# maelaubert/VulkanSift

Hardware: AMD Instinct MI355X
Metric: SIFT detect+match frames/sec (640x480, ~2k kp) (higher is better)
Workload: dtype f32

## Files before the change

include/vksift_hip.h:

```cpp
#ifndef VKSIFT_HIP_H
#define VKSIFT_HIP_H

#include <stddef.h>
#include <stdint.h>

#ifdef __cplusplus
extern "C"
{
#endif

#define VKSIFT_HIP_MAX_TAPS 20
#define VKSIFT_HIP_MATCH_CHUNKS 32
#define VKSIFT_HIP_MATCH_SMALL_NA 1536u
#define VKSIFT_HIP_MATCH_SMALL_NB 4096u
#define VKSIFT_HIP_MATCH_SCRATCH_U32(na, nb) (2u * (size_t)(na) + (size_t)(nb) + 72u + (size_t)(na) * 16u * VKSIFT_HIP_MATCH_CHUNKS)
#define VKSIFT_HIP_ABI_VERSION 14u
#define VKSIFT_HIP_GATHER_SLOTS 512u
#define VKSIFT_HIP_MATCH_SLOTS 256u
#define VKSIFT_HIP_MATCH_PK_NB 32768u
#define VKSIFT_HIP_MAX_ORI 18
#define VKSIFT_HIP_MAX_OCTAVE_SIDE 16383u

  typedef void *vksift_hip_stream;
  typedef void *vksift_hip_graph;
  typedef void *vksift_hip_event;

  int vksift_hip_init(void);
  uint32_t vksift_hip_abi_version(void);
  int vksift_hip_device_count(void);
  int vksift_hip_device_name(int idx, char *out256);
  int vksift_hip_set_device(int idx);
  size_t vksift_hip_device_free_mem(void);
  void *vksift_hip_malloc(size_t bytes);
  void vksift_hip_free(void *p);
  void *vksift_hip_host_malloc(size_t bytes);
  void vksift_hip_host_free(void *p);
  int vksift_hip_host_register(void *p, size_t bytes);
  int vksift_hip_host_unregister(void *p);
  int vksift_hip_is_pinned(const void *p);
  vksift_hip_stream vksift_hip_stream_create(void);
  void vksift_hip_stream_destroy(vksift_hip_stream s);
  int vksift_hip_stream_sync(vksift_hip_stream s);
  int vksift_hip_stream_busy(vksift_hip_stream s);
  vksift_hip_event vksift_hip_event_create(void);
  void vksift_hip_event_destroy(vksift_hip_event e);
  int vksift_hip_event_record(vksift_hip_event e, vksift_hip_stream s);
  int vksift_hip_event_sync(vksift_hip_event e);
  int vksift_hip_event_busy(vksift_hip_event e);
  float vksift_hip_event_elapsed_ms(vksift_hip_event a, vksift_hip_event b);
  int vksift_hip_stream_wait_event(vksift_hip_stream s, vksift_hip_event e);
  int vksift_hip_capture_begin(vksift_hip_stream s);
  int vksift_hip_capture_end(vksift_hip_stream s, vksift_hip_graph *out);
  int vksift_hip_graph_launch(vksift_hip_graph g, vksift_hip_stream s);
  void vksift_hip_graph_destroy(vksift_hip_graph g);
  int vksift_hip_memcpy_h2d(void *dst, const void *src, size_t n, vksift_hip_stream s);
  int vksift_hip_memcpy_d2h(void *dst, const void *src, size_t n, vksift_hip_stream s);
  int vksift_hip_memcpy_d2d(void *dst, const void *src, size_t n, vksift_hip_stream s);
  int vksift_hip_memcpy2d_d2h(void *dst, size_t dpitch, const void *src, size_t spitch, size_t width_bytes, size_t height, vksift_hip_stream s);
  int vksift_hip_post_words(uint32_t *host_mapped_dst, const uint32_t *src, size_t n_words, vksift_hip_stream s);
  int vksift_hip_memset(void *dst, int value, size_t n, vksift_hip_stream s);
  const char *vksift_hip_error_string(int err);
  void vksift_hip_range_push(const char *name);
  void vksift_hip_range_pop(void);

  enum
  {
    VKSIFT_TUNE_WG_TARGET = 0,
    VKSIFT_TUNE_WIDE_MASK = 1,
    VKSIFT_TUNE_MULTI_MAX = 2,
    VKSIFT_TUNE_REFINE_PTR = 3,
    VKSIFT_TUNE_SCAN_FORM = 4,
    VKSIFT_TUNE_PAIR_FORM = 5,
    VKSIFT_TUNE_PYR_GATE = 6,
    VKSIFT_TUNE_DENSE_ROWS = 7,
    VKSIFT_TUNE_SEED_WG = 8,
    VKSIFT_TUNE_SCAN_BAND = 9,
    VKSIFT_TUNE_TAIL_MULTI = 10,
    VKSIFT_TUNE_ZERO_COPY = 11,
    VKSIFT_TUNE_MIN_MARCH = 12,
    VKSIFT_TUNE_TAIL_FUSED = 13,
    VKSIFT_TUNE_COUNT = 16
  };
  int vksift_hip_tune(int knob, int value);
  int vksift_hip_tune_get(int knob);


  typedef struct
  {
    float *base;
    uint32_t w, h;
    uint32_t pitch;
    uint64_t img_stride;
    uint32_t fp16;
    uint32_t reverse;
  } vksift_hip_Plane;

  int vksift_hip_input_blit(const uint8_t *src, uint32_t sw, uint32_t sh, uint64_t src_img_stride, vksift_hip_Plane dst, uint32_t batch,
                            vksift_hip_stream s);

  int vksift_hip_blur(vksift_hip_Plane src, vksift_hip_Plane dst, const float *taps, uint32_t ntaps, uint32_t batch, vksift_hip_stream s);

  int vksift_hip_blur_pair(vksift_hip_Plane src, vksift_hip_Plane dst1, vksift_hip_Plane dst2, const float *taps1, uint32_t ntaps1, const float *taps2,
                           uint32_t ntaps2, uint32_t batch, vksift_hip_stream s);

  int vksift_hip_blur_form(vksift_hip_Plane src, vksift_hip_Plane dst, uint32_t ntaps, uint32_t batch);

  int vksift_hip_blur_multi(const vksift_hip_Plane *src, const vksift_hip_Plane *dst, uint32_t n, const float *taps, uint32_t ntaps, uint32_t batch,
                            vksift_hip_stream s);

  int vksift_hip_blur_downsample(vksift_hip_Plane src, vksift_hip_Plane dst, vksift_hip_Plane next, const float *taps, uint32_t ntaps, uint32_t batch,
                                 vksift_hip_stream s);

  int vksift_hip_seed_upsampled(const uint8_t *src, uint32_t sw, uint32_t sh, uint64_t src_img_stride, vksift_hip_Plane dst, const float *taps, uint32_t ntaps,
                                uint32_t batch, vksift_hip_stream s);

  int vksift_hip_seed_direct(const uint8_t *src, uint32_t sw, uint32_t sh, uint64_t src_img_stride, vksift_hip_Plane dst, const float *taps, uint32_t ntaps,
                             uint32_t batch, vksift_hip_stream s);

  int vksift_hip_downsample(vksift_hip_Plane src, vksift_hip_Plane dst, uint32_t batch, vksift_hip_stream s);

  int vksift_hip_octave_chain(const vksift_hip_Plane *layers, uint32_t n_oct, uint32_t n_layers, uint32_t S, const float *taps, const uint32_t *ntaps,
                              uint32_t batch, vksift_hip_stream s);

  int vksift_hip_dog_plane(const float *lo, const float *hi, uint32_t w, uint32_t h, uint32_t pitch, uint32_t fp16, float *out_dense, vksift_hip_stream s);

  typedef struct
  {
    float *gauss;
    uint32_t fp16;
    uint32_t w, h, pitch;
    uint64_t plane_stride;
    uint64_t img_stride;
    uint32_t S;
    int32_t octave_idx;
    float seed_sigma;
    float dog_threshold;
    float edge_limit;
    uint8_t *feats;
    uint64_t feat_img_stride;
    uint32_t cap;
    uint32_t *found;
    uint32_t found_img_stride;
    uint64_t *seg_mask;
    uint32_t *seg_off;
    uint64_t seg_img_stride;
    uint32_t *cand_xy;
    uint32_t *cand_flag;
    uint32_t *cand_n;
    uint64_t cand_img_stride;
    uint32_t cand_cap;
    float *ori_ang;
    uint32_t *ori_cnt;
    uint64_t ori_img_stride;
    uint32_t max_ori;
    uint32_t use_vlfeat;
    const float *desc_fp_tab;
    uint32_t desc_fp_tab_len;
    uint32_t scan_reverse;
    uint32_t masks_cleared;
    uint32_t sec_index;
  } vksift_hip_OctaveJob;

  typedef struct
  {
    uint8_t *desc;
    uint64_t desc_img_stride;
    uint32_t *norm;
    uint64_t norm_img_stride;
    uint32_t *n;
    uint32_t n_img_stride;
    uint32_t nsec;
    uint32_t sec_cap[16];
    uint8_t *post;
    uint64_t post_img_stride;
    uint32_t *found_post;
    uint32_t found_post_n;
  } vksift_hip_DenseRows;

  int vksift_hip_extract_keypoints(const vksift_hip_OctaveJob *job, uint32_t batch, vksift_hip_stream s, vksift_hip_event scan_done);
  int vksift_hip_orientations(const vksift_hip_OctaveJob *job, uint32_t batch, vksift_hip_stream s);
  int vksift_hip_descriptors(const vksift_hip_OctaveJob *job, uint32_t batch, vksift_hip_stream s);
  int vksift_hip_extract_keypoints_multi(const vksift_hip_OctaveJob *jobs, uint32_t n_jobs, uint32_t batch, vksift_hip_stream s, vksift_hip_event scan_done);
  int vksift_hip_clear_segment_masks(const vksift_hip_OctaveJob *jobs, uint32_t n_jobs, uint32_t batch, vksift_hip_stream s);
  int vksift_hip_selftest_inrange(uint32_t n, uint32_t seed, uint32_t *d_mismatches, vksift_hip_stream s);
  int vksift_hip_orientations_multi(const vksift_hip_OctaveJob *jobs, uint32_t n_jobs, uint32_t batch, vksift_hip_stream s);
  int vksift_hip_descriptors_multi(const vksift_hip_OctaveJob *jobs, uint32_t n_jobs, uint32_t batch, vksift_hip_stream s);
  int vksift_hip_descriptors_multi_dense(const vksift_hip_OctaveJob *jobs, uint32_t n_jobs, uint32_t batch, const vksift_hip_DenseRows *dense,
                                         vksift_hip_stream s);

  typedef struct
  {
    float x, y, sigma, orientation, response;
  } vksift_hip_Keypoint;
  typedef struct
  {
    uint32_t w, h;
    int32_t octave_idx;
    uint8_t *feats;
    uint64_t feat_img_stride;
    uint32_t cap;
    uint32_t *found;
    uint32_t found_img_stride;
  } vksift_hip_PlaceOctave;
#define VKSIFT_HIP_PLACE_WG 256u
  int vksift_hip_place_keypoints(const vksift_hip_Keypoint *kps, const uint32_t *kp_first, const vksift_hip_PlaceOctave *oct, uint32_t n_oct,
                                 const float *sigma_steps, uint32_t S, uint32_t keep_orientation, uint32_t batch, uint32_t *placed, vksift_hip_stream s);

  int vksift_hip_gather_descriptors(const uint8_t *feats, uint32_t n, uint8_t *desc, vksift_hip_stream s);
  size_t vksift_hip_match_scratch_u32(uint32_t na, uint32_t nb);
  int vksift_hip_match_2nn_desc(const uint8_t *desc_a, uint32_t na, uint32_t a_index_base, const uint8_t *desc_b, uint32_t nb, uint32_t *norm_scratch,
                                size_t scratch_u32, uint8_t *matches, vksift_hip_stream s);
  int vksift_hip_shifted_norms(const uint8_t *desc, uint32_t n, uint32_t *norms, vksift_hip_stream s);
  int vksift_hip_match_2nn_prenormed(const uint8_t *desc_a, const uint32_t *norm_a, uint32_t na, uint32_t a_index_base, const uint8_t *desc_b,
                                     const uint32_t *norm_b, uint32_t nb, uint32_t *scratch, size_t scratch_u32, uint8_t *matches, vksift_hip_stream s);

  int vksift_hip_filter_matches(const uint8_t *fwd, uint64_t fwd_slot_stride, const uint8_t *rev, uint64_t rev_slot_stride, const uint32_t *n_fwd,
                                uint32_t n_stride, float ratio, uint32_t nslots, uint8_t *out, uint64_t out_slot_stride, uint32_t *out_n, vksift_hip_stream s);

  int vksift_hip_pack_features(const uint8_t *feats_base, uint64_t buf_stride, const uint32_t *buf_ids, const uint32_t *out_rows, uint32_t nslots, uint32_t nsec,
                               const uint32_t *sec_off, const uint32_t *sec_cap, const uint32_t *found_base, uint32_t found_buf_stride, uint8_t *out,
                               uint32_t max_rows, uint32_t *found_post, vksift_hip_stream s);
  int vksift_hip_gather_sections(const uint8_t *feats_base, uint64_t buf_stride, const uint32_t *buf_ids, uint32_t nslots, uint32_t nsec,
                                 const uint32_t *sec_off, const uint32_t *sec_cap, const uint32_t *fixed_counts, const uint32_t *found_base,
                                 uint32_t found_buf_stride, uint32_t max_rows, uint32_t pad_rows_to, uint8_t *desc, uint64_t desc_stride,
                                 uint32_t *norms, uint64_t norm_stride, uint32_t *n_out_dev, uint32_t n_stride, vksift_hip_stream s);
  int vksift_hip_keep_strongest(uint8_t *feats_base, uint64_t buf_stride, const uint32_t *buf_ids, uint32_t nslots, uint32_t nsec, const uint32_t *sec_off,
                                const uint32_t *sec_cap, const uint32_t *fixed_counts, uint32_t *found_base, uint32_t found_buf_stride, uint32_t *found_post,
                                uint32_t max_features, uint32_t pad_rows_to, uint8_t *desc, uint64_t desc_stride, uint32_t *norms, uint64_t norm_stride,
                                uint32_t *n_out_dev, uint32_t n_stride, vksift_hip_stream s);
  int vksift_hip_keep_grid(uint8_t *feats_base, uint64_t buf_stride, const uint32_t *buf_ids, uint32_t nslots, uint32_t nsec, const uint32_t *sec_off,
                           const uint32_t *sec_cap, const uint32_t *fixed_counts, uint32_t *found_base, uint32_t found_buf_stride, uint32_t *found_post,
                           uint32_t max_features, uint32_t grid_cols, uint32_t grid_rows, const float *col_bounds, const float *row_bounds,
                           uint32_t pad_rows_to, uint8_t *desc, uint64_t desc_stride, uint32_t *norms, uint64_t norm_stride, uint32_t *n_out_dev,
                           uint32_t n_stride, vksift_hip_stream s);
  int vksift_hip_root_descriptors(uint8_t *feats_base, uint64_t buf_stride, const uint32_t *buf_ids, uint32_t nslots, uint32_t nsec, const uint32_t *sec_off,
// ... 59 lines not shown
```

vulkansift_amd/csrc/hip/features.hip:

```cpp
#include <hip/hip_runtime.h>
#include <stdint.h>
#include <stdlib.h>
#include <type_traits>

#include "../detmath.h"
#include "features_math.h"
#include "multi.h"
#include "records.h"
#include "vksift_hip.h"
#include "wave.h"

namespace
{

struct FeatArgs
{
  const float *gauss;
  uint32_t fp16;
  int w, h, pitch;
  uint64_t plane_stride, img_stride;
  uint8_t *feats;
  uint64_t feat_img_stride;
  uint32_t cap;
  uint32_t *found;
// ... 167 lines not shown
      }
      uint32_t hm = __shfl(hv, lm, 64), hp = __shfl(hv, lp, 64);
      const uint32_t mx = wave_max_u32(lane < 36 ? hv : 0u);
      bool peak = lane < 36 && ((float)hv >= (0.8f * (float)mx)) && (hv > hm) && (hv > hp);
      unsigned long long pm = __ballot(peak);
      uint32_t npk = (uint32_t)__popcll(pm);
      if (peak)
      {
        uint32_t rank = ballot_rank(pm, lane);
        if (rank < a.max_keep)
        {
          uint32_t num = hm - hp;
          uint32_t den = hm - (2u * hv) + hp;
          float idx = (float)lane + 0.5f * ((float)num / (float)den);
          float ang = (idx + 0.5f) * (2.f * PI_F) / 36.f;
          a.ori_ang[((size_t)b * a.ori_img_stride + k) * VKSIFT_HIP_MAX_ORI + rank] = ang;
        }
      }
      if (lane == 0)
        a.ori_cnt[(size_t)b * a.ori_img_stride + k] = npk < a.max_keep ? npk : a.max_keep;
    }
    __builtin_amdgcn_wave_barrier();
  }
}

__global__ void __launch_bounds__(1024) k_orientation_finalize(Multi<FeatArgs> m)
{
  __shared__ uint32_t wave_tot[16];
  __shared__ uint32_t carry_s;
  const VBlock vb = vblock(m);
  const FeatArgs &a = m.oct[vb.o];
  const int b = (int)vb.x;
  const int lane = threadIdx.x & 63, wave = threadIdx.x >> 6;
  const ImageView g = image_view(a, b);
  const uint32_t *cnt = a.ori_cnt + (size_t)b * a.ori_img_stride;
  const float *ang = a.ori_ang + (size_t)b * a.ori_img_stride * VKSIFT_HIP_MAX_ORI;
  if (threadIdx.x == 0)
    carry_s = 0;
  __syncthreads();
  for (uint32_t base = 0; base < g.n; base += 1024)
  {
    uint32_t k = base + threadIdx.x;
    uint32_t c = k < g.n ? cnt[k] : 0u;
    uint32_t v = c > 1 ? c - 1 : 0u;
    const uint32_t incl = wave_scan_incl_u32(v, lane);
    if (lane == 63)
      wave_tot[wave] = incl;
    __syncthreads();
    uint32_t wave_base = 0;
    for (int wv = 0; wv < wave; wv++)
      wave_base += wave_tot[wv];
    uint32_t carry = carry_s;
    uint32_t excl = carry + wave_base + incl - v;
    if (k < g.n && c >= 1)
    {
      uint32_t *rec = (uint32_t *)(g.feats + (size_t)k * VKSIFT_RECORD_BYTES);
      rec[7] = __float_as_uint(ang[(size_t)k * VKSIFT_HIP_MAX_ORI]);
      for (uint32_t j = 1; j < c; j++)
      {
        uint32_t idx = g.found + excl + (j - 1);
        if (idx < a.cap)
        {
          uint32_t *dst = (uint32_t *)(g.feats + (size_t)idx * VKSIFT_RECORD_BYTES);
#pragma unroll
          for (int q = 0; q < (int)VKSIFT_RECORD_HEAD_WORDS; q++)
            dst[q] = rec[q];
          dst[7] = __float_as_uint(ang[(size_t)k * VKSIFT_HIP_MAX_ORI + j]);
        }
      }
    }
    __syncthreads();
    if (threadIdx.x == 1023)
      carry_s = carry + wave_base + incl;
    __syncthreads();
  }
  if (threadIdx.x == 0)
    a.found[(size_t)b * a.found_img_stride] = g.found + carry_s;
}

__device__ __forceinline__ int smod8(int v) { return v & 7; }

struct DescCtx
{
  __amdgpu_buffer_rsrc_t rs;
  int pitch, pitch4;
  float scale_x, scale_y, rsx, rsy, kcos, ksin, kori, fp, bin_scale;
  int dx0, dx1, dy0, dy1;
  float offx, offy, ia0, ia1;
};

struct DescSample
{
  float ox, oy, mag;
  float xb;
};

struct DescTaps
{
  float up, lf, rt, dn;
};

__device__ __forceinline__ unsigned desc_tap_base(const DescCtx &c, int cdx, int cdy)
{
  const int ix = (int)c.rsx + cdx, iy = (int)c.rsy + cdy;
  return (__umul24((unsigned)(iy - 1), (unsigned)c.pitch) + (unsigned)(ix - 1)) * 4u;
}

template <bool F16>
__device__ __forceinline__ DescTaps desc_taps(const DescCtx &c, unsigned v0)
{
  DescTaps t;
  t.up = tap_ld<F16>(c.rs, v0 + 4u, 0);
  t.lf = tap_ld<F16>(c.rs, v0, c.pitch4);
  t.rt = tap_ld<F16>(c.rs, v0 + 8u, c.pitch4);
  t.dn = tap_ld<F16>(c.rs, v0 + 4u, 2 * c.pitch4);
  return t;
}

typedef uint32_t u32x2_t __attribute__((ext_vector_type(2)));
typedef uint32_t u32x4_t __attribute__((ext_vector_type(4)));
__device__ __forceinline__ void desc_taps_pair(const DescCtx &c, unsigned v0, DescTaps &a, DescTaps &b)
{
  const u32x2_t up = __builtin_amdgcn_raw_buffer_load_b64(c.rs, v0 + 4u, 0, 0);
  const u32x4_t mid = __builtin_amdgcn_raw_buffer_load_b128(c.rs, v0, c.pitch4, 0);
  const u32x2_t dn = __builtin_amdgcn_raw_buffer_load_b64(c.rs, v0 + 4u, 2 * c.pitch4, 0);
  a.up = __uint_as_float(up.x), b.up = __uint_as_float(up.y);
  a.lf = __uint_as_float(mid.x), b.lf = __uint_as_float(mid.y);
  a.rt = __uint_as_float(mid.z), b.rt = __uint_as_float(mid.w);
  a.dn = __uint_as_float(dn.x), b.dn = __uint_as_float(dn.y);
}

template <bool INRANGE>
__device__ __forceinline__ DescSample desc_sample(const DescCtx &c, int cdx, int cdy, const DescTaps &t, bool *odd)
{
  const float es = -1.f / (2.f * 2 * 2);
  float sdx = (c.rsx + (float)cdx) - c.scale_x;
  float sdy = (c.rsy + (float)cdy) - c.scale_y;
  DescSample r;
  r.ox = c.kcos * sdx + c.ksin * sdy;
  r.oy = c.kcos * sdy - c.ksin * sdx;
  float gradX = 0.5f * (t.rt - t.lf);
  float gradY = 0.5f * (t.dn - t.up);
  float ori, root;
  grad_polar<INRANGE>(gradX, gradY, &ori, &root, odd);
  ori = wrap_2pi(ori);
  ori = wrap_2pi(ori - c.kori);
  r.mag = dm_expf_core_nonpos(es * ((r.ox * r.ox) + (r.oy * r.oy))) * root;
  r.xb = ori * c.bin_scale;
  return r;
}

constexpr int DESC_PAD = 1, DESC_ROW_CELLS = 8;
constexpr int DESC_HIST_WORDS = (4 + 2 * DESC_PAD) * DESC_ROW_CELLS * 16;
constexpr int DESC_WORK_WORDS = DESC_HIST_WORDS;
__device__ __forceinline__ int desc_cell_word(int cell)
{
  return (((cell >> 2) + DESC_PAD) * DESC_ROW_CELLS + (cell & 3) + DESC_PAD) * 16;
}
__device__ __forceinline__ uint32_t desc_hist_read(const uint32_t *s_work, int t)
{
  const int cw = desc_cell_word(t >> 3), bin = t & 7;
  return s_work[cw + 2 * bin] + s_work[cw + 2 * ((bin + 7) & 7) + 1];
}

__device__ __forceinline__ void desc_scatter(const DescCtx &c, const DescSample &r, float fbin, bool live, uint32_t *s_work)
{
  float fhx = r.ox + 2.f, fhy = r.oy + 2.f;
  const float flx = floorf(fhx - 0.5f), fly = floorf(fhy - 0.5f), flb = floorf(fbin);
  int hx = (int)flx, hy = (int)fly, hb = (int)flb;
  float rhx = fhx - (flx + 0.5f), rhy = fhy - (fly + 0.5f), rb = fbin - flb;
  const float magfp = r.mag * c.fp;
  const unsigned b0 = (unsigned)smod8(hb);
  const unsigned pair = b0 * 8u;
  const bool okx[2] = {live && (unsigned)hx < 4u, live && (unsigned)(hx + 1) < 4u};
  const bool oky[2] = {(unsigned)hy < 4u, (unsigned)(hy + 1) < 4u};
  char *base = (char *)s_work + ((unsigned)((hy + DESC_PAD) * (DESC_ROW_CELLS * 64) + (hx + DESC_PAD) * 64) + pair);
#pragma unroll
  for (int i = 0; i < 2; i++)
#pragma unroll
    for (int j = 0; j < 2; j++)
    {
      const float w = fabsf(1.f - (float)i - rhx) * fabsf(1.f - (float)j - rhy);
      const uint32_t v0 = (uint32_t)((w * fabsf(1.f - 0.f - rb)) * magfp);
      const uint32_t v1 = (uint32_t)((w * fabsf(1.f - 1.f - rb)) * magfp);
      if (okx[i] && oky[j])
        atomicAdd((unsigned long long *)(base + (j * DESC_ROW_CELLS * 64 + i * 64)), ((unsigned long long)v1 << 32) | v0);
    }
}

constexpr int DESC_MAX_ROWS = 256;

template <bool CAN_POST>
__device__ __forceinline__ void desc_dense_prologue(const FeatArgs &a, const vksift_hip_DenseRows &dr, int b, bool first_block, int tid, uint32_t *s_row0)
{
  if (!(dr.desc || (CAN_POST && dr.post)))
    return;
  const uint32_t *fsec = a.found + (size_t)b * a.found_img_stride - a.sec;
  uint32_t row0 = 0, total = 0;
#pragma unroll
  for (uint32_t j = 0; j < 16u; j++)
    if (j < dr.nsec)
    {
      const uint32_t f = fsec[j], n = f < dr.sec_cap[j] ? f : dr.sec_cap[j];
      row0 += j < a.sec ? n : 0u;
      total += n;
    }
  if (tid == 0)
    *s_row0 = row0;
  if (a.sec == 0 && first_block)
  {
    if (CAN_POST && dr.post && (uint32_t)tid < dr.found_post_n)
      dr.found_post[(size_t)b * dr.found_post_n + tid] = fsec[tid];
    if (dr.desc && tid == 0)
      dr.n[(size_t)b * dr.n_img_stride] = total;
    if (dr.desc && total < 2u && tid < 64)
    {
      uint32_t *z = (uint32_t *)(dr.desc + (size_t)b * dr.desc_img_stride);
      if (tid >= (int)total * 32)
        z[tid] = 0u;
      if (tid < 2 && tid >= (int)total)
        dr.norm[(size_t)b * dr.norm_img_stride + tid] = 128u * 128u * 128u;
    }
  }
}

__device__ __forceinline__ DescCtx desc_setup(const FeatArgs &a, const ImageView &g, const KeyHead &kh)
{
  DescCtx c;
  c.scale_x = kh.scale_x, c.scale_y = kh.scale_y, c.kori = kh.theta;
  c.rs = kh.rs;
  c.pitch = g.pitch, c.pitch4 = g.pitch * 4;
  c.bin_scale = a.use_vlfeat ? 8.f : -8.f;
  float scale_factor = dm_pow2i(kh.octave_idx);
  float lambda = 3.0f * (kh.sigma / scale_factor);
  float radius = sqrtf(2.f) * lambda * 5.f * 0.5f;
  int R = (int)floorf(radius + 0.5f);
  float sn, cs;
  dm_sincosf(c.kori, &sn, &cs);
  c.kcos = cs / lambda, c.ksin = sn / lambda;
  uint32_t ti = (uint32_t)(R / 2);
  c.fp = a.desc_fp_tab[ti < a.desc_fp_tab_len ? ti : a.desc_fp_tab_len - 1];
  c.rsx = roundf(c.scale_x), c.rsy = roundf(c.scale_y);

  const int cxi = (int)c.rsx, cyi = (int)c.rsy;
  c.dx0 = max(-R, 1 - cxi), c.dx1 = min(R, g.w - 2 - cxi);
  c.dy0 = max(-R, 1 - cyi), c.dy1 = min(R, g.h - 2 - cyi);
  c.offx = c.rsx - c.scale_x, c.offy = c.rsy - c.scale_y;
  c.ia0 = __builtin_amdgcn_rcpf(c.kcos), c.ia1 = __builtin_amdgcn_rcpf(-c.ksin);
  return c;
}

struct DescRows
{
  int *lo;
  uint32_t *cnt;
  const uint32_t *pre;
  int y0, nrows;
};

template <int NT>
__device__ __forceinline__ void desc_row_spans(const DescCtx &c, const DescRows &rows, int tid)
{
  const float T = 2.5f + 0.01f;
  for (int row = tid; row < rows.nrows; row += NT)
  {
    const float fy = (float)(rows.y0 + row) + c.offy;
    float lo = (float)c.dx0 - 0.5f, hi = (float)c.dx1 + 0.5f;
#pragma unroll
    for (int e = 0; e < 2; e++)
    {
      const float aa = e == 0 ? c.kcos : -c.ksin, ia = e == 0 ? c.ia0 : c.ia1;
      const float bb = e == 0 ? c.ksin * fy : c.kcos * fy;
      if (fabsf(aa) > 1e-12f)
      {
        const float ctr = -bb * ia - c.offx, half = T * fabsf(ia);
        lo = fmaxf(lo, ctr - half);
        hi = fminf(hi, ctr + half);
      }
      else if (!(fabsf(bb) < T))
        hi = lo - 2.f;
    }
    const int ilo = (int)ceilf(lo - 0.01f), ihi = (int)floorf(hi + 0.01f);
    const int xl = max(ilo, c.dx0), xh = min(ihi, c.dx1);
    rows.lo[row] = xl;
    rows.cnt[row] = xh >= xl ? (uint32_t)(xh - xl + 1) : 0u;
  }
}

__device__ __forceinline__ void desc_row_prefix(const DescRows &rows, uint32_t *pre, int lane)
{
  uint32_t carry = 0;
  for (int base = 0; base < rows.nrows; base += 64)
  {
    const int i = base + lane;
    const uint32_t v = i < rows.nrows ? rows.cnt[i] : 0u;
    const uint32_t incl = wave_scan_incl_u32(v, lane);
    if (i < rows.nrows)
      pre[i] = carry + incl - v;
    carry += __shfl(incl, 63, 64);
  }
  if (lane == 0)
    pre[rows.nrows] = carry;
}

struct DescRun
{
  uint32_t steps;
  uint32_t sidx, send;
  int row, cdx;
  uint32_t row_end;
};
template <int NWV>
__device__ __forceinline__ DescRun desc_run(const DescRows &rows, int wave, int lane)
{
  const uint32_t *s_pre = rows.pre;
  const uint32_t N = s_pre[rows.nrows];
  const uint32_t T = (N + 63u) / 64u, tq = T / NWV, tr = T % NWV;
  DescRun r;
  r.steps = tq + ((uint32_t)wave < tr ? 1u : 0u);
  const uint32_t step0 = (uint32_t)wave * tq + min((uint32_t)wave, tr);
  r.sidx = min(N, step0 * 64u + (uint32_t)lane * r.steps);
  r.send = min(N, r.sidx + r.steps);
  int row = 0;
  if (r.sidx < r.send)
  {
    int lo_r = 0, hi_r = rows.nrows - 1;
    while (lo_r < hi_r)
    {
      const int mid = (lo_r + hi_r + 1) >> 1;
      if (s_pre[mid] <= r.sidx)
        lo_r = mid;
      else
        hi_r = mid - 1;
    }
    row = lo_r;
    while (s_pre[row + 1] <= r.sidx)
      row++;
  }
  r.row = row;
  r.cdx = rows.lo[row] + (int)(r.sidx - s_pre[row]);
  r.row_end = s_pre[row + 1];
  return r;
}

__device__ __forceinline__ bool desc_next_sample(const DescRows &rows, DescRun &r, int &sx, int &sy)
{
  const bool live = r.sidx < r.send;
  if (live && r.sidx >= r.row_end)
  {
    do
      r.row++;
    while (rows.pre[r.row + 1] <= r.sidx);
    r.row_end = rows.pre[r.row + 1];
    r.cdx = rows.lo[r.row];
  }
  sx = r.cdx, sy = rows.y0 + r.row;
  r.cdx++, r.sidx++;
  return live;
}

template <bool F16>
__device__ __forceinline__ void desc_step_pair(const DescCtx &c, const DescRows &rows, DescRun &run, uint32_t *s_work)
{
  int sx[2], sy[2];
  const bool live[2] = {desc_next_sample(rows, run, sx[0], sy[0]), desc_next_sample(rows, run, sx[1], sy[1])};
  DescTaps t0, t1;
  const unsigned v0 = desc_tap_base(c, sx[0], sy[0]);
  if (F16)
  {
    t0 = desc_taps<F16>(c, v0);
    t1 = desc_taps<F16>(c, desc_tap_base(c, sx[1], sy[1]));
  }
  else
  {
    desc_taps_pair(c, v0, t0, t1);
    if (live[1] && !(sy[1] == sy[0] && sx[1] == sx[0] + 1))
      t1 = desc_taps<F16>(c, desc_tap_base(c, sx[1], sy[1]));
  }
  bool o0, o1;
  DescSample s0 = desc_sample<true>(c, sx[0], sy[0], t0, &o0), s1 = desc_sample<true>(c, sx[1], sy[1], t1, &o1);
  float f0 = angle_bin<true>(s0.xb), f1 = angle_bin<true>(s1.xb);
  o0 |= angle_bin_odd(s0.xb), o1 |= angle_bin_odd(s1.xb);
  if (__builtin_expect(__ballot(o0 || o1) != 0ull, 0))
  {
    s0 = desc_sample<false>(c, sx[0], sy[0], t0, nullptr), s1 = desc_sample<false>(c, sx[1], sy[1], t1, nullptr);
    f0 = angle_bin<false>(s0.xb), f1 = angle_bin<false>(s1.xb);
  }
  desc_scatter(c, s0, f0, live[0], s_work);
  desc_scatter(c, s1, f1, live[1], s_work);
}

template <bool F16>
__device__ __forceinline__ void desc_step_odd(const DescCtx &c, const DescRows &rows, DescRun &run, uint32_t *s_work)
{
  int sx, sy;
  const bool live = desc_next_sample(rows, run, sx, sy);
  const DescSample s0 = desc_sample<false>(c, sx, sy, desc_taps<F16>(c, desc_tap_base(c, sx, sy)), nullptr);
  desc_scatter(c, s0, angle_bin<false>(s0.xb), live, s_work);
}

__device__ __forceinline__ uint32_t desc_byte(float v) { return (v != v) ? 0u : (v < 0.f ? 0u : (v > 255.f ? 255u : (uint32_t)v)); }
__device__ __forceinline__ void desc_bytes(const uint32_t *s_work, int ln, uint32_t &b0, uint32_t &b1)
{
  uint32_t w0 = desc_hist_read(s_work, ln), w1 = desc_hist_read(s_work, ln + 64);
  float norm = sqrtf((float)wave_sum_u32(w0 * w0 + w1 * w1));
  uint32_t lim = (uint32_t)(norm * 0.2f);
  w0 = w0 < lim ? w0 : lim;
  w1 = w1 < lim ? w1 : lim;
  norm = sqrtf((float)wave_sum_u32(w0 * w0 + w1 * w1));
  float scale = 512.f / norm;
  b0 = desc_byte((float)w0 * scale), b1 = desc_byte((float)w1 * scale);
}
__device__ __forceinline__ uint32_t desc_pack4(uint32_t byte, int ln)
{
  uint32_t p = byte << ((uint32_t)(ln & 3) * 8u);
  p |= __shfl_xor(p, 1, 64);
  p |= __shfl_xor(p, 2, 64);
  return p;
}
__device__ __forceinline__ void desc_store_dwords(uint32_t *dst, int ln, uint32_t p0, uint32_t p1)
{
  if ((ln & 3) == 0)
  {
    dst[ln >> 2] = p0;
    dst[16 + (ln >> 2)] = p1;
  }
}
__device__ __forceinline__ void desc_post_record(const vksift_hip_DenseRows &dr, int b, uint32_t row, const float *rec, int ln, uint32_t p0, uint32_t p1)
{
  const uint32_t j = (uint32_t)ln & 15u;
  const uint32_t d0 = __shfl(p0, (int)(4u * j), 64), d1 = __shfl(p1, (int)(4u * j), 64);
  uint32_t *out = (uint32_t *)(dr.post + (size_t)b * dr.post_img_stride) + (size_t)row * VKSIFT_RECORD_WORDS;
  if (ln < 32)
    out[(int)VKSIFT_RECORD_HEAD_WORDS + ln] = ln < 16 ? d0 : d1;
  else if (ln < (int)VKSIFT_RECORD_WORDS)
    out[ln - 32] = ((const uint32_t *)rec)[ln - 32];
}
__device__ __forceinline__ void desc_dense_row(const vksift_hip_DenseRows &dr, int b, uint32_t row0, uint32_t k, int ln, uint32_t p0, uint32_t p1)
{
  uint32_t *dense = (uint32_t *)(dr.desc + (size_t)b * dr.desc_img_stride) + (size_t)row0 * 32;
  uint32_t *dense_norm = dr.norm + (size_t)b * dr.norm_img_stride + row0;
  uint32_t s2 = __builtin_amdgcn_udot4(p0, p0, 0u, false), s1 = __builtin_amdgcn_udot4(p0, 0x01010101u, 0u, false);
  s2 = __builtin_amdgcn_udot4(p1, p1, s2, false), s1 = __builtin_amdgcn_udot4(p1, 0x01010101u, s1, false);
#pragma unroll
  for (int dlt = 32; dlt >= 4; dlt >>= 1)
  {
    s2 += __shfl_xor(s2, dlt, 64);
    s1 += __shfl_xor(s1, dlt, 64);
  }
  desc_store_dwords(dense + (size_t)k * 32, ln, p0, p1);
  if (ln == 0)
    dense_norm[k] = s2 - 256u * s1 + 128u * 128u * 128u;
}

template <bool CAN_POST>
__device__ __forceinline__ void desc_epilogue(const vksift_hip_DenseRows &dr, const ImageView &g, int b, uint32_t k, const float *rec, const uint32_t *s_work,
                                              const uint32_t *s_row0, int lane)
{
  int ln = lane;
  asm volatile("" : "+v"(ln));
  uint32_t b0, b1;
  desc_bytes(s_work, ln, b0, b1);
  const uint32_t p0 = desc_pack4(b0, ln), p1 = desc_pack4(b1, ln);
  desc_store_dwords((uint32_t *)(g.feats + (size_t)k * VKSIFT_RECORD_BYTES + VKSIFT_RECORD_DESC_AT), ln, p0, p1);
  if (CAN_POST && dr.post)
    desc_post_record(dr, b, *s_row0 + k, rec, ln, p0, p1);
  if (dr.desc)
    desc_dense_row(dr, b, *s_row0, k, ln, p0, p1);
}

template <int NWV, bool IMG_FAST, bool F16>
__global__ void __launch_bounds__(64 * NWV) __attribute__((amdgpu_waves_per_eu((NWV == 2 && !F16) ? 8 : 6, 8)))
k_descriptor(Multi<FeatArgs> m, vksift_hip_DenseRows dr)
{
  const VBlock vb = vblock(m);
  const FeatArgs &a = m.oct[vb.o];
  constexpr int NT_ = 64 * NWV;
  __shared__ __attribute__((aligned(8))) uint32_t s_work[DESC_WORK_WORDS];
  __shared__ int s_row_lo[DESC_MAX_ROWS];
  __shared__ uint32_t s_row_cnt[DESC_MAX_ROWS];
  __shared__ uint32_t s_row_pre[NWV][DESC_MAX_ROWS + 1];
  __shared__ uint32_t s_row0;
  const int tid = threadIdx.x, lane = threadIdx.x & 63, wave = threadIdx.x >> 6;
  const int b = (int)(IMG_FAST ? vb.x : vb.y);
  const ImageView g = image_view(a, b);
  const uint32_t bk = IMG_FAST ? vb.y : vb.x, nbk = IMG_FAST ? vb.gy : vb.gx;
  constexpr bool CAN_POST = NWV == 4;
  desc_dense_prologue<CAN_POST>(a, dr, b, bk == 0, tid, &s_row0);

  for (uint32_t k = bk; k < g.n; k += nbk)
  {
    __syncthreads();
    for (int i = tid; i < 256; i += NT_)
      s_work[desc_cell_word(i >> 4) + (i & 15)] = 0;

    const KeyHead kh = keypoint_head<F16>(a, g, b, k);
    const DescCtx c = desc_setup(a, g, kh);
    const int bh = c.dy1 - c.dy0 + 1;
    for (int rb = 0; rb < bh; rb += DESC_MAX_ROWS)
    {
      const DescRows rows{s_row_lo, s_row_cnt, s_row_pre[wave], c.dy0 + rb, min(DESC_MAX_ROWS, bh - rb)};
      __syncthreads();
      desc_row_spans<NT_>(c, rows, tid);
      __syncthreads();
      desc_row_prefix(rows, s_row_pre[wave], lane);
      __builtin_amdgcn_wave_barrier();
      DescRun run = desc_run<NWV>(rows, wave, lane);
      uint32_t it = 0;
      for (; it + 1 < run.steps; it += 2)
        desc_step_pair<F16>(c, rows, run, s_work);
      if (it < run.steps)
        desc_step_odd<F16>(c, rows, run, s_work);
    }
    __syncthreads();
    if (wave == 0)
      desc_epilogue<CAN_POST>(dr, g, b, k, kh.rec, s_work, &s_row0, lane);
  }
}

FeatArgs make_args(const vksift_hip_OctaveJob *job)
{
  FeatArgs a;
  a.gauss = job->gauss;
  a.fp16 = job->fp16;
  a.w = (int)job->w, a.h = (int)job->h, a.pitch = (int)job->pitch;
  a.plane_stride = job->plane_stride, a.img_stride = job->img_stride;
  a.feats = job->feats, a.feat_img_stride = job->feat_img_stride, a.cap = job->cap;
  a.found = job->found, a.found_img_stride = job->found_img_stride;
  a.ori_ang = job->ori_ang, a.ori_cnt = job->ori_cnt, a.ori_img_stride = job->ori_img_stride;
  uint32_t mk = job->max_ori == 0 ? VKSIFT_HIP_MAX_ORI : job->max_ori;
  a.max_keep = mk > VKSIFT_HIP_MAX_ORI ? VKSIFT_HIP_MAX_ORI : mk;
  a.use_vlfeat = job->use_vlfeat;
  a.desc_fp_tab = job->desc_fp_tab, a.desc_fp_tab_len = job->desc_fp_tab_len;
  a.sec = job->sec_index;
  return a;
}

bool img_fast(uint32_t batch, bool descriptor)
{
  return batch > 1 && !descriptor;
}

bool add_octave(Multi<FeatArgs> &m, const FeatArgs &a, bool img_fast, uint32_t batch, uint32_t blocks)
{
  return multi_add(m, a, img_fast ? batch : blocks, img_fast ? blocks : batch, 1u);
}

uint32_t expected_keypoints(const vksift_hip_OctaveJob *job, uint32_t batch)
{
  const uint32_t pixels_per_keypoint = 512;
  if (batch < 8u)
    return 0xFFFFFFFFu;
  const uint64_t n = (uint64_t)job->w * job->h / pixels_per_keypoint;
  return n < 32u ? 32u : (n > 0xFFFFFFFFull ? 0xFFFFFFFFu : (uint32_t)n);
}

uint32_t octave_blocks(const vksift_hip_OctaveJob *job, uint32_t batch, uint32_t kp_per_block, uint32_t cap_blocks)
{
  const uint32_t dense = expected_keypoints(job, batch);
  uint32_t blocks = ((job->cap < dense ? job->cap : dense) + (kp_per_block - 1)) / kp_per_block;
  if (blocks > cap_blocks)
    blocks = cap_blocks;
  return blocks == 0 ? 1 : blocks;
}

}

static int orientation_run(const vksift_hip_OctaveJob *jobs, uint32_t n, uint32_t batch, hipStream_t hs)
{
  Multi<FeatArgs> mo, mf;
  mo.n = mf.n = 0;
  const bool f = img_fast(batch, false);
  uint32_t cap_blocks = 16384u / batch;
  cap_blocks = cap_blocks < 32u ? 32u : (cap_blocks > 1024u ? 1024u : cap_blocks);
  for (uint32_t i = 0; i < n; i++)
  {
    const FeatArgs a = make_args(&jobs[i]);
    if (!add_octave(mo, a, f, batch, octave_blocks(&jobs[i], batch, 4, cap_blocks)) || !multi_add(mf, a, batch, 1u, 1u))
      return (int)hipErrorInvalidValue;
  }
  const bool f16 = mo.oct[0].fp16 != 0;
  const dim3 grid(mo.start[mo.n]);
  with_bool(f, [&](auto IMG_FAST) {
    with_bool(f16, [&](auto F16) { hipLaunchKernelGGL((k_orientation<decltype(IMG_FAST)::value, decltype(F16)::value>), grid, dim3(256), 0, hs, mo); });
  });
  hipLaunchKernelGGL(k_orientation_finalize, dim3(mf.start[mf.n]), dim3(1024), 0, hs, mf);
  return (int)hipGetLastError();
}

static int descriptor_run(const vksift_hip_OctaveJob *jobs, uint32_t n, uint32_t batch, const vksift_hip_DenseRows &dr, hipStream_t hs)
{
  Multi<FeatArgs> md;
  md.n = 0;
  const bool f = img_fast(batch, true);
  for (uint32_t i = 0; i < n; i++)
    if (!add_octave(md, make_args(&jobs[i]), f, batch, octave_blocks(&jobs[i], batch, 1, 2048)))
      return (int)hipErrorInvalidValue;
  const bool two_waves = batch >= 8u;
  if (dr.post && two_waves)
    return (int)hipErrorInvalidValue;
  const bool f16 = md.oct[0].fp16 != 0;
  const dim3 grid(md.start[md.n]);
  with_bool(two_waves, [&](auto TWO) {
    constexpr int NWV = decltype(TWO)::value ? 2 : 4;
    with_bool(f, [&](auto IMG_FAST) {
      with_bool(f16, [&](auto F16) {
        hipLaunchKernelGGL((k_descriptor<NWV, decltype(IMG_FAST)::value, decltype(F16)::value>), grid, dim3(64 * NWV), 0, hs, md, dr);
      });
    });
  });
  return (int)hipGetLastError();
}

template <typename F>
static int for_runs(const vksift_hip_OctaveJob *jobs, uint32_t n_jobs, F run)
{
  for (uint32_t i0 = 0; i0 < n_jobs;)
  {
    uint32_t i1 = i0 + 1;
    while (i1 < n_jobs && i1 - i0 < multi_run_max() && jobs[i1].fp16 == jobs[i0].fp16)
      i1++;
    const int e = run(jobs + i0, i1 - i0);
    if (e)
      return e;
    i0 = i1;
  }
  return 0;
}

extern "C"
{
  int vksift_hip_orientations_multi(const vksift_hip_OctaveJob *jobs, uint32_t n_jobs, uint32_t batch, vksift_hip_stream s)
  {
    if (batch == 0)
      return 0;
    return for_runs(jobs, n_jobs, [&](const vksift_hip_OctaveJob *j, uint32_t n) { return orientation_run(j, n, batch, (hipStream_t)s); });
  }

  int vksift_hip_descriptors_multi_dense(const vksift_hip_OctaveJob *jobs, uint32_t n_jobs, uint32_t batch, const vksift_hip_DenseRows *dense,
                                         vksift_hip_stream s)
  {
    if (batch == 0)
      return 0;
    vksift_hip_DenseRows dr = {};
    if (dense)
    {
      const bool rows = dense->desc != NULL, post = dense->post != NULL;
      if ((!rows && !post) || (rows && (!dense->norm || !dense->n)) || (post && (!dense->found_post || dense->found_post_n > 64u)) || dense->nsec == 0 ||
          dense->nsec > 16u)
        return (int)hipErrorInvalidValue;
      for (uint32_t i = 0; i < n_jobs; i++)
        if (jobs[i].sec_index >= dense->nsec)
          return (int)hipErrorInvalidValue;
      dr = *dense;
    }
    return for_runs(jobs, n_jobs, [&](const vksift_hip_OctaveJob *j, uint32_t n) { return descriptor_run(j, n, batch, dr, (hipStream_t)s); });
  }

  int vksift_hip_descriptors_multi(const vksift_hip_OctaveJob *jobs, uint32_t n_jobs, uint32_t batch, vksift_hip_stream s)
  {
    return vksift_hip_descriptors_multi_dense(jobs, n_jobs, batch, nullptr, s);
  }

  int vksift_hip_orientations(const vksift_hip_OctaveJob *job, uint32_t batch, vksift_hip_stream s) { return vksift_hip_orientations_multi(job, 1, batch, s); }

  int vksift_hip_descriptors(const vksift_hip_OctaveJob *job, uint32_t batch, vksift_hip_stream s) { return vksift_hip_descriptors_multi(job, 1, batch, s); }
}
```

vulkansift_amd/csrc/hip/runtime.hip:

```cpp
#include <hip/hip_runtime.h>
#include <roctracer/roctx.h>

#include <cstdio>
#include <cstring>

#include "vksift_hip.h"

__global__ void k_post_words(uint32_t *__restrict__ dst, const uint32_t *__restrict__ src, unsigned long long n)
{
  const unsigned long long i = (unsigned long long)blockIdx.x * blockDim.x + threadIdx.x;
  if (i < n)
    dst[i] = src[i];
}

extern "C"
{

  uint32_t vksift_hip_abi_version(void) { return VKSIFT_HIP_ABI_VERSION; }

  static int g_tune[VKSIFT_TUNE_COUNT] = {0, -1, 0, 0, 0, 0, 0, 0, 0, 0, 0, 0, 0, 0, 0, 0};
  int vksift_hip_tune(int knob, int value)
  {
    if (knob < 0 || knob >= VKSIFT_TUNE_COUNT)
      return -1;
    g_tune[knob] = value;
    return 0;
  }
  int vksift_hip_tune_get(int knob) { return (knob >= 0 && knob < VKSIFT_TUNE_COUNT) ? g_tune[knob] : 0; }

  int vksift_hip_init(void)
  {
    hipError_t e = hipInit(0);
    if (e != hipSuccess)
      return (int)e;
    int n = 0;
    e = hipGetDeviceCount(&n);
    if (e != hipSuccess)
      return (int)e;
    return n > 0 ? 0 : (int)hipErrorNoDevice;
  }

  int vksift_hip_device_count(void)
  {
    int n = 0;
    if (hipGetDeviceCount(&n) != hipSuccess)
      return 0;
    return n;
  }

  int vksift_hip_device_name(int idx, char *out256)
  {
    hipDeviceProp_t prop;
    hipError_t e = hipGetDeviceProperties(&prop, idx);
    if (e != hipSuccess)
      return (int)e;
    std::memset(out256, 0, 256);
    std::snprintf(out256, 256, "%s (%s)", prop.name, prop.gcnArchName);
    return 0;
  }

  int vksift_hip_set_device(int idx) { return (int)hipSetDevice(idx); }

  size_t vksift_hip_device_free_mem(void)
  {
    size_t f = 0, t = 0;
    if (hipMemGetInfo(&f, &t) != hipSuccess)
      return 0;
    return f;
  }

  void *vksift_hip_malloc(size_t bytes)
  {
    void *p = nullptr;
    if (hipMalloc(&p, bytes ? bytes : 1) != hipSuccess)
      return nullptr;
    return p;
  }
  void vksift_hip_free(void *p)
  {
    if (p)
      (void)hipFree(p);
  }
  void *vksift_hip_host_malloc(size_t bytes)
  {
    void *p = nullptr;
    if (hipHostMalloc(&p, bytes ? bytes : 1, hipHostMallocDefault) != hipSuccess)
      return nullptr;
    return p;
  }
  int vksift_hip_host_register(void *p, size_t bytes) { return (int)hipHostRegister(p, bytes, hipHostRegisterDefault); }
  int vksift_hip_host_unregister(void *p) { return (int)hipHostUnregister(p); }
  int vksift_hip_is_pinned(const void *p)
  {
    hipPointerAttribute_t a;
    if (hipPointerGetAttributes(&a, p) != hipSuccess)
    {
      (void)hipGetLastError();
      return 0;
    }
    return a.type == hipMemoryTypeHost ? 1 : 0;
  }

  void vksift_hip_host_free(void *p)
  {
    if (p)
      (void)hipHostFree(p);
  }

  vksift_hip_stream vksift_hip_stream_create(void)
  {
    hipStream_t s = nullptr;
    if (hipStreamCreateWithFlags(&s, hipStreamNonBlocking) != hipSuccess)
      return nullptr;
    return (vksift_hip_stream)s;
  }
  void vksift_hip_stream_destroy(vksift_hip_stream s)
  {
    if (s)
      (void)hipStreamDestroy((hipStream_t)s);
  }
  int vksift_hip_stream_sync(vksift_hip_stream s) { return (int)hipStreamSynchronize((hipStream_t)s); }
  int vksift_hip_stream_busy(vksift_hip_stream s)
  {
    hipError_t e = hipStreamQuery((hipStream_t)s);
    if (e == hipSuccess)
      return 0;
    if (e == hipErrorNotReady)
      return 1;
    return -(int)e;
  }

  vksift_hip_event vksift_hip_event_create(void)
  {
    hipEvent_t e = nullptr;
    if (hipEventCreate(&e) != hipSuccess)
      return nullptr;
    return (vksift_hip_event)e;
  }
  void vksift_hip_event_destroy(vksift_hip_event e)
  {
    if (e)
      (void)hipEventDestroy((hipEvent_t)e);
  }
  int vksift_hip_event_record(vksift_hip_event e, vksift_hip_stream s) { return (int)hipEventRecord((hipEvent_t)e, (hipStream_t)s); }
  int vksift_hip_event_sync(vksift_hip_event e) { return (int)hipEventSynchronize((hipEvent_t)e); }
  int vksift_hip_event_busy(vksift_hip_event e)
  {
    hipError_t r = hipEventQuery((hipEvent_t)e);
    if (r == hipSuccess)
      return 0;
    if (r == hipErrorNotReady)
      return 1;
    return -(int)r;
  }
  float vksift_hip_event_elapsed_ms(vksift_hip_event a, vksift_hip_event b)
  {
    float ms = -1.f;
    if (hipEventElapsedTime(&ms, (hipEvent_t)a, (hipEvent_t)b) != hipSuccess)
      return -1.f;
    return ms;
  }
  int vksift_hip_stream_wait_event(vksift_hip_stream s, vksift_hip_event e) { return (int)hipStreamWaitEvent((hipStream_t)s, (hipEvent_t)e, 0); }

  int vksift_hip_capture_begin(vksift_hip_stream s) { return (int)hipStreamBeginCapture((hipStream_t)s, hipStreamCaptureModeRelaxed); }
  int vksift_hip_capture_end(vksift_hip_stream s, vksift_hip_graph *out)
  {
    hipGraph_t g = nullptr;
    hipGraphExec_t ge = nullptr;
    *out = nullptr;
    hipError_t e = hipStreamEndCapture((hipStream_t)s, &g);
    if (e != hipSuccess)
      return (int)e;
    e = hipGraphInstantiate(&ge, g, nullptr, nullptr, 0);
// ... 45 lines not shown
```

Baseline: 25900.

## Process small-radius keypoint pairs with one wave each in descriptor kernel

In the two-wave descriptor kernel, each block now takes pairs of keypoints. When both keypoints have a window radius at or below a tunable limit, each wave builds one descriptor on its own, using wave-level barriers, a private histogram buffer and half of the row arrays. Larger pairs fall back to the old path where both waves cooperate on one keypoint. This cuts block-wide syncs and gives more parallel work for small keypoints, at the cost of an extra histogram buffer in LDS, a per-pair radius check, and uneven load between waves.

```diff
diff --git a/include/vksift_hip.h b/include/vksift_hip.h
--- a/include/vksift_hip.h
+++ b/include/vksift_hip.h
@@ -79,8 +79,10 @@
     VKSIFT_TUNE_ZERO_COPY = 11,
     VKSIFT_TUNE_MIN_MARCH = 12,
     VKSIFT_TUNE_TAIL_FUSED = 13,
+    VKSIFT_TUNE_DESC_SOLO_R = 14,
     VKSIFT_TUNE_COUNT = 16
   };
+#define VKSIFT_HIP_DESC_SOLO_R 63
   int vksift_hip_tune(int knob, int value);
   int vksift_hip_tune_get(int knob);
 
diff --git a/vulkansift_amd/csrc/hip/features.hip b/vulkansift_amd/csrc/hip/features.hip
--- a/vulkansift_amd/csrc/hip/features.hip
+++ b/vulkansift_amd/csrc/hip/features.hip
@@ -343,7 +343,8 @@
 
 constexpr int DESC_PAD = 1, DESC_ROW_CELLS = 8;
 constexpr int DESC_HIST_WORDS = (4 + 2 * DESC_PAD) * DESC_ROW_CELLS * 16;
-constexpr int DESC_WORK_WORDS = DESC_HIST_WORDS;
+constexpr int DESC_WORK_WORDS = ((4 + DESC_PAD - 1) * DESC_ROW_CELLS + (4 + DESC_PAD - 1) + 1) * 16;
+static_assert(DESC_WORK_WORDS <= DESC_HIST_WORDS && DESC_WORK_WORDS % 2 == 0, "64-bit slots");
 __device__ __forceinline__ int desc_cell_word(int cell)
 {
   return (((cell >> 2) + DESC_PAD) * DESC_ROW_CELLS + (cell & 3) + DESC_PAD) * 16;
@@ -415,6 +416,14 @@
   }
 }
 
+__device__ __forceinline__ int desc_radius(float sigma, int octave_idx, float *lambda)
+{
+  float scale_factor = dm_pow2i(octave_idx);
+  *lambda = 3.0f * (sigma / scale_factor);
+  float radius = sqrtf(2.f) * *lambda * 5.f * 0.5f;
+  return (int)floorf(radius + 0.5f);
+}
+
 __device__ __forceinline__ DescCtx desc_setup(const FeatArgs &a, const ImageView &g, const KeyHead &kh)
 {
   DescCtx c;
@@ -422,10 +431,8 @@
   c.rs = kh.rs;
   c.pitch = g.pitch, c.pitch4 = g.pitch * 4;
   c.bin_scale = a.use_vlfeat ? 8.f : -8.f;
-  float scale_factor = dm_pow2i(kh.octave_idx);
-  float lambda = 3.0f * (kh.sigma / scale_factor);
-  float radius = sqrtf(2.f) * lambda * 5.f * 0.5f;
-  int R = (int)floorf(radius + 0.5f);
+  float lambda;
+  const int R = desc_radius(kh.sigma, kh.octave_idx, &lambda);
   float sn, cs;
   dm_sincosf(c.kori, &sn, &cs);
   c.kcos = cs / lambda, c.ksin = sn / lambda;
@@ -660,52 +667,108 @@
     desc_dense_row(dr, b, *s_row0, k, ln, p0, p1);
 }
 
-template <int NWV, bool IMG_FAST, bool F16>
-__global__ void __launch_bounds__(64 * NWV) __attribute__((amdgpu_waves_per_eu((NWV == 2 && !F16) ? 8 : 6, 8)))
-k_descriptor(Multi<FeatArgs> m, vksift_hip_DenseRows dr)
-{
-  const VBlock vb = vblock(m);
-  const FeatArgs &a = m.oct[vb.o];
-  constexpr int NT_ = 64 * NWV;
-  __shared__ __attribute__((aligned(8))) uint32_t s_work[DESC_WORK_WORDS];
-  __shared__ int s_row_lo[DESC_MAX_ROWS];
-  __shared__ uint32_t s_row_cnt[DESC_MAX_ROWS];
-  __shared__ uint32_t s_row_pre[NWV][DESC_MAX_ROWS + 1];
-  __shared__ uint32_t s_row0;
-  const int tid = threadIdx.x, lane = threadIdx.x & 63, wave = threadIdx.x >> 6;
-  const int b = (int)(IMG_FAST ? vb.x : vb.y);
-  const ImageView g = image_view(a, b);
-  const uint32_t bk = IMG_FAST ? vb.y : vb.x, nbk = IMG_FAST ? vb.gy : vb.gx;
-  constexpr bool CAN_POST = NWV == 4;
-  desc_dense_prologue<CAN_POST>(a, dr, b, bk == 0, tid, &s_row0);
-
-  for (uint32_t k = bk; k < g.n; k += nbk)
-  {
+template <int NW>
+__device__ __forceinline__ void desc_sync()
+{
+  if (NW == 1)
+    __builtin_amdgcn_wave_barrier();
+  else
     __syncthreads();
-    for (int i = tid; i < 256; i += NT_)
+}
+template <int NW, int NPH, int MAXR, bool PAIRS, bool CAN_POST, bool F16>
+__device__ __forceinline__ void desc_keypoint(const FeatArgs &a, const vksift_hip_DenseRows &dr, const ImageView &g, int b, uint32_t k, int wave, int tid,
+                                              uint32_t *s_work, int *s_lo, uint32_t *s_cnt, uint32_t *s_pre, const uint32_t *s_row0)
+{
+  desc_sync<NW>();
+  {
+    int zt = tid;
+    if (PAIRS)
+      asm volatile("" : "+v"(zt));
+    for (int i = zt; i < 256; i += 64 * NW)
       s_work[desc_cell_word(i >> 4) + (i & 15)] = 0;
-
-    const KeyHead kh = keypoint_head<F16>(a, g, b, k);
-    const DescCtx c = desc_setup(a, g, kh);
-    const int bh = c.dy1 - c.dy0 + 1;
-    for (int rb = 0; rb < bh; rb += DESC_MAX_ROWS)
+  }
+
+  const KeyHead kh = keypoint_head<F16>(a, g, b, k);
+  const DescCtx c = desc_setup(a, g, kh);
+  const int bh = c.dy1 - c.dy0 + 1;
+  for (int rb = 0; rb < bh; rb += MAXR)
+  {
+    const DescRows rows{s_lo, s_cnt, s_pre, c.dy0 + rb, min(MAXR, bh - rb)};
+    int rt = tid;
+    if (PAIRS)
+      asm volatile("" : "+v"(rt));
+    desc_sync<NW>();
+    desc_row_spans<64 * NW>(c, rows, rt);
+    desc_sync<NW>();
+    desc_row_prefix(rows, s_pre, rt & 63);
+    __builtin_amdgcn_wave_barrier();
+#pragma unroll 1
+    for (int ph = 0; ph < NPH; ph++)
     {
-      const DescRows rows{s_row_lo, s_row_cnt, s_row_pre[wave], c.dy0 + rb, min(DESC_MAX_ROWS, bh - rb)};
-      __syncthreads();
-      desc_row_spans<NT_>(c, rows, tid);
-      __syncthreads();
-      desc_row_prefix(rows, s_row_pre[wave], lane);
-      __builtin_amdgcn_wave_barrier();
-      DescRun run = desc_run<NWV>(rows, wave, lane);
+      int pt = tid;
+      if (PAIRS)
+        asm volatile("" : "+v"(pt));
+      DescRun run = desc_run<NW * NPH>(rows, wave * NPH + ph, pt & 63);
       uint32_t it = 0;
       for (; it + 1 < run.steps; it += 2)
         desc_step_pair<F16>(c, rows, run, s_work);
       if (it < run.steps)
         desc_step_odd<F16>(c, rows, run, s_work);
     }
+  }
+  desc_sync<NW>();
+  if (wave == 0)
+    desc_epilogue<CAN_POST>(dr, g, b, k, kh.rec, s_work, s_row0, tid & 63);
+}
+
+#ifndef DESC_SOLO_PHASES
+#define DESC_SOLO_PHASES 4
+#endif
+constexpr int DESC_SOLO_MAX_R = 63;
+__device__ __forceinline__ bool desc_pair_small(const ImageView &g, uint32_t k0, int lane, uint32_t solo_r)
+{
+  const float *rec = (const float *)(g.feats + (size_t)(k0 + ((uint32_t)lane & 1u)) * VKSIFT_RECORD_BYTES);
+  float lambda;
+  const int R = desc_radius(rec[6], ((const int *)rec)[5], &lambda);
+  return __ballot(R > (int)solo_r) == 0ull;
+}
+
+template <int NWV, bool IMG_FAST, bool F16>
+__global__ void __launch_bounds__(64 * NWV) __attribute__((amdgpu_waves_per_eu((NWV == 2 && !F16) ? 8 : 6, 8)))
+k_descriptor(Multi<FeatArgs> m, vksift_hip_DenseRows dr, uint32_t solo_r)
+{
+  const VBlock vb = vblock(m);
+  const FeatArgs &a = m.oct[vb.o];
+  constexpr int NSOLO = NWV == 2 ? 2 : 1;
+  static_assert(2 * DESC_SOLO_MAX_R + 1 <= DESC_MAX_ROWS / 2, "a solo window's rows fit half of the row arrays");
+  __shared__ __attribute__((aligned(8))) uint32_t s_work[NSOLO][DESC_WORK_WORDS];
+  __shared__ int s_row_lo[DESC_MAX_ROWS];
+  __shared__ uint32_t s_row_cnt[DESC_MAX_ROWS];
+  __shared__ uint32_t s_row_pre[NWV][DESC_MAX_ROWS + 1];
+  __shared__ uint32_t s_row0;
+  const int tid = threadIdx.x, lane = threadIdx.x & 63, wave = __builtin_amdgcn_readfirstlane(threadIdx.x >> 6);
+  const int b = (int)(IMG_FAST ? vb.x : vb.y);
+  const ImageView g = image_view(a, b);
+  const uint32_t bk = IMG_FAST ? vb.y : vb.x, nbk = IMG_FAST ? vb.gy : vb.gx;
+  constexpr bool CAN_POST = NWV == 4;
+  desc_dense_prologue<CAN_POST>(a, dr, b, bk == 0, tid, &s_row0);
+
+  const uint32_t per = (NWV == 2 && solo_r != 0u) ? 2u : 1u;
+  if (per == 2u)
     __syncthreads();
-    if (wave == 0)
-      desc_epilogue<CAN_POST>(dr, g, b, k, kh.rec, s_work, &s_row0, lane);
+  for (uint32_t k0 = bk * per; k0 < g.n; k0 += nbk * per)
+  {
+    if constexpr (NWV == 2)
+      if (per == 2u && k0 + 1u < g.n && desc_pair_small(g, k0, lane, solo_r))
+      {
+        constexpr int HALF = DESC_MAX_ROWS / 2;
+        desc_keypoint<1, DESC_SOLO_PHASES, HALF, true, CAN_POST, F16>(a, dr, g, b, k0 + (uint32_t)wave, 0, lane, s_work[wave], s_row_lo + wave * HALF, s_row_cnt + wave * HALF,
+                                              s_row_pre[wave], &s_row0);
+        continue;
+      }
+    const uint32_t k1 = min(k0 + per, g.n);
+    for (uint32_t k = k0; k < k1; k++)
+      desc_keypoint<NWV, 1, DESC_MAX_ROWS, NWV == 2, CAN_POST, F16>(a, dr, g, b, k, wave, tid, s_work[0], s_row_lo, s_row_cnt, s_row_pre[wave], &s_row0);
   }
 }
 
@@ -784,10 +847,12 @@
   Multi<FeatArgs> md;
   md.n = 0;
   const bool f = img_fast(batch, true);
+  const bool two_waves = batch >= 8u;
+  const int tune_r = vksift_hip_tune_get(VKSIFT_TUNE_DESC_SOLO_R);
+  const uint32_t solo_r = !two_waves || tune_r <= 0 ? 0u : (tune_r > DESC_SOLO_MAX_R ? (uint32_t)DESC_SOLO_MAX_R : (uint32_t)tune_r);
   for (uint32_t i = 0; i < n; i++)
-    if (!add_octave(md, make_args(&jobs[i]), f, batch, octave_blocks(&jobs[i], batch, 1, 2048)))
+    if (!add_octave(md, make_args(&jobs[i]), f, batch, octave_blocks(&jobs[i], batch, solo_r ? 2 : 1, 2048)))
       return (int)hipErrorInvalidValue;
-  const bool two_waves = batch >= 8u;
   if (dr.post && two_waves)
     return (int)hipErrorInvalidValue;
   const bool f16 = md.oct[0].fp16 != 0;
@@ -796,7 +861,7 @@
     constexpr int NWV = decltype(TWO)::value ? 2 : 4;
     with_bool(f, [&](auto IMG_FAST) {
       with_bool(f16, [&](auto F16) {
-        hipLaunchKernelGGL((k_descriptor<NWV, decltype(IMG_FAST)::value, decltype(F16)::value>), grid, dim3(64 * NWV), 0, hs, md, dr);
+        hipLaunchKernelGGL((k_descriptor<NWV, decltype(IMG_FAST)::value, decltype(F16)::value>), grid, dim3(64 * NWV), 0, hs, md, dr, solo_r);
       });
     });
   });
diff --git a/vulkansift_amd/csrc/hip/runtime.hip b/vulkansift_amd/csrc/hip/runtime.hip
--- a/vulkansift_amd/csrc/hip/runtime.hip
+++ b/vulkansift_amd/csrc/hip/runtime.hip
@@ -18,7 +18,7 @@
 
   uint32_t vksift_hip_abi_version(void) { return VKSIFT_HIP_ABI_VERSION; }
 
-  static int g_tune[VKSIFT_TUNE_COUNT] = {0, -1, 0, 0, 0, 0, 0, 0, 0, 0, 0, 0, 0, 0, 0, 0};
+  static int g_tune[VKSIFT_TUNE_COUNT] = {0, -1, 0, 0, 0, 0, 0, 0, 0, 0, 0, 0, 0, 0, VKSIFT_HIP_DESC_SOLO_R, 0};
   int vksift_hip_tune(int knob, int value)
   {
     if (knob < 0 || knob >= VKSIFT_TUNE_COUNT)
```

After: 26450, median of 6. +2.1%, better.
